# artis-mcrt/artis

Measured on AMD Instinct MI355X. Metric: packet-steps/sec, higher is better.
Workload: dtype f64

## Files before the change

### artis_amd/csrc/artis_engine.hip

```cpp
#include <hip/hip_runtime.h>
#include <rccl/rccl.h>

#include <dlfcn.h>

#include <cstdio>
#include <cstdlib>
#include <algorithm>
#include <chrono>
#include <cstring>
#include <string>
#include <type_traits>
#include <utility>
#include <vector>
#include <cmath>

#include "model_build.h"
#include "engine_config.h"
#include "physics.h"
#include "radfield_fit.h"
#include "ion_balance.h"
#include "spectra.h"

#include <rocprim/device/device_radix_sort.hpp>

// ... 91 lines not shown
  int base = 0;
  for (int w0 = 0; w0 < nw; w0 += 64) {
    const int j = w0 + lane;
    unsigned long long word = (j < nw) ? keep[j] : 0ull;
    const int pc = __popcll(word);
    int incl = pc;
#pragma unroll
    for (int o = 1; o < 64; o <<= 1) {
      const int v = __shfl_up(incl, o);
      if (lane >= o) incl += v;
    }
    int at = base + incl - pc;
    if (j < nw) prefix[j] = at;
    while (word != 0ull) {
      const int i = (j * 64) + __builtin_ctzll(word);
      list[at] = i;
      keptpair[at] = pair[i];
      at++;
      word &= word - 1ull;
    }
    base += __shfl(incl, 63);
  }
}
__global__ void __launch_bounds__(BLOCK) k_corrphotoion(Env env, const int32_t *target_level) {
  const int64_t i = (int64_t)blockIdx.x * BLOCK + threadIdx.x;
  const int64_t total = fill_count(env) * env.M.nphixstargets_total;
  if (i >= total) return;
  const int c = fill_cell(env, i / env.M.nphixstargets_total);
  const int k = (int)(i % env.M.nphixstargets_total);
  const int ul = target_level[k];
  populate_corrphotoion(env, c, ul, k - env.M.level_phixstargetstart[ul]);
}
__device__ inline double wave_shr1(double x) {
  int lo = __double2loint(x), hi = __double2hiint(x);
  lo = __builtin_amdgcn_update_dpp(0, lo, 0x138 , 0xF, 0xF, false);
  hi = __builtin_amdgcn_update_dpp(0, hi, 0x138, 0xF, 0xF, false);
  return __hiloint2double(hi, lo);
}
__device__ inline unsigned long long line_lanes(int lane, int ti, int seglen) {
  const int first = lane - (ti % MAREC_PER);
  const int left = seglen - (ti - (ti % MAREC_PER));
  const int cnt = left < MAREC_PER ? left : MAREC_PER;
  return ((1ull << cnt) - 1ull) << first;
}
struct MaEntryPos {
  LevelPack lpk;
  int ti, seglen, e_seg0;
  bool isdown;
};
__device__ inline MaEntryPos ma_entry_pos(const DevModel &M, int a0, int e) {
  MaEntryPos r;
  r.lpk = M.level_pack[M.alltrans_owner[a0 + e]];
  const int i = (a0 + e) - r.lpk.alltrans_startdown;
  r.isdown = i < r.lpk.ndown;
  r.ti = r.isdown ? i : i - r.lpk.ndown;
  r.seglen = r.isdown ? r.lpk.ndown : r.lpk.nup;
  r.e_seg0 = e - r.ti;
  return r;
}
__global__ void __launch_bounds__(BLOCK, 4) k_matrans(Env env) {
  __shared__ double lds_v[BLOCK / 64][3][MATRANS_BLOCK];
  __shared__ uint16_t lds_q[BLOCK / 64][2][MATRANS_BLOCK];
  __shared__ uint8_t lds_qf[BLOCK / 64][MATRANS_BLOCK];
  __shared__ uint8_t lds_ok[BLOCK / 64][2][MATRANS_BLOCK];
  const int64_t wave = ((int64_t)blockIdx.x * BLOCK + threadIdx.x) >> 6;
  const int lane = threadIdx.x & 63, w = threadIdx.x >> 6;
  const DevModel &M = env.M;
  const int nblk = M.nscanblk;
  if (wave >= fill_count(env) * nblk) return;
  const int64_t kf = wave / nblk;
  const int c = fill_cell(env, kf);
  const int blk = (int)(wave % nblk);
  const int seg0 = M.scanblk_seg0[blk], seg1 = M.scanblk_seg0[blk + 1];
  const MaLongSeg sfirst = M.scansegs[seg0], slast = M.scansegs[seg1 - 1];
  const int a0 = sfirst.ats0, nent = (slast.ats0 + slast.n) - a0;
  U4 *row = env.K.macache + (krow(env, c) * M.nmacache);
  double *upterms = env.collexc_terms + (kf * M.nupcum);
  double(*v)[MATRANS_BLOCK] = lds_v[w];
  if (nent > MATRANS_BLOCK) {
    const LevelPack lpk = M.level_pack[sfirst.ul];
    double c0 = 0., c1 = 0., c2 = 0.;
    for (int base = 0; base < nent; base += 64) {
      const bool valid = base + lane < nent;
      MaTransTerms t;
      t.v0 = t.v1 = t.v2 = t.kterm = 0.;
      if (valid) {
        t = matrans_terms<ARTIS_COLD_COOLING_ONLY != 0>(env, c, a0 + base + lane);
        if (!t.isdown) upterms[M.level_upcum_start[t.ul] + t.i] = t.kterm;
      }
      double s0 = (lane == 0 ? c0 : 0.) + t.v0, s1 = (lane == 0 ? c1 : 0.) + t.v1, s2 = (lane == 0 ? c2 : 0.) + t.v2;
      for (int k = 1; k < 64; k++) {
        const double p0 = wave_shr1(s0), p1 = wave_shr1(s1), p2 = wave_shr1(s2);
        if (lane == k) {
          s0 = p0 + t.v0;
          s1 = p1 + t.v1;
          s2 = p2 + t.v2;
        }
      }
      const int last = (nent - base < 64 ? nent - base : 64) - 1;
      c0 = __shfl(s0, last);
      c1 = __shfl(s1, last);
      c2 = __shfl(s2, last);
    }
    if (lane == 0 && lpk.rec_off >= 0) {
      double *rates = ma_rates_of(row + lpk.rec_off, lpk.ndown, lpk.nup);
      if (sfirst.dir == 0) {
        rates[ARTIS_MA_ACTION_RADDEEXC] = c0;
        rates[ARTIS_MA_ACTION_COLDEEXC] = c1;
        rates[ARTIS_MA_ACTION_INTERNALDOWNSAME] = c2;
      } else {
        rates[ARTIS_MA_ACTION_INTERNALUPSAME] = c0;
      }
    }
    return;
  }
  for (int k = lane; k < nent; k += 64) {
    const int e = M.scanperm[a0 + k];
    const MaTransTerms t = matrans_terms<ARTIS_COLD_COOLING_ONLY != 0>(env, c, a0 + e);
    v[0][e] = t.v0;
    v[1][e] = t.v1;
    v[2][e] = t.v2;
    lds_ok[w][0][e] = 1;
    lds_ok[w][1][e] = 1;
    if (!t.isdown) upterms[M.level_upcum_start[t.ul] + t.i] = t.kterm;
  }
  __threadfence_block();
  for (int si = seg0 + lane; si < seg1; si += 64) {
    const MaLongSeg sg = M.scansegs[si];
    const int o = sg.ats0 - a0;
    double s0 = 0., s1 = 0., s2 = 0.;
    for (int i = 0; i < sg.n; i++) {
      s0 += v[0][o + i];
      s1 += v[1][o + i];
      s2 += v[2][o + i];
      v[0][o + i] = s0;
      v[2][o + i] = s2;
    }
    const LevelPack lpk = M.level_pack[sg.ul];
    if (lpk.rec_off < 0) continue;
    double *rates = ma_rates_of(row + lpk.rec_off, lpk.ndown, lpk.nup);
    if (sg.dir == 0) {
      rates[ARTIS_MA_ACTION_RADDEEXC] = s0;
      rates[ARTIS_MA_ACTION_COLDEEXC] = s1;
      rates[ARTIS_MA_ACTION_INTERNALDOWNSAME] = s2;
    } else {
      rates[ARTIS_MA_ACTION_INTERNALUPSAME] = s0;
    }
  }
  __threadfence_block();
  for (int e = lane; e < nent; e += 64) {
    const MaEntryPos ps = ma_entry_pos(M, a0, e);
    const int e_last = ps.e_seg0 + ps.seglen - 1;
    const double whole_int = v[ps.isdown ? 2 : 0][e_last], whole_rad = v[0][e_last];
    bool ok_int = (whole_int > 0.) && (whole_int <= DBLMAX), ok_rad = (whole_rad > 0.) && (whole_rad <= DBLMAX);
    uint32_t q_int = MAFILT_NONE23, q_rad = MAFILT_NONE;
    if (ps.ti < ps.seglen - 1) {
      if (ok_int) q_int = mafilt_quant23(v[ps.isdown ? 2 : 0][e], whole_int, &ok_int);
      if (ok_rad && ps.isdown) q_rad = mafilt_quant(v[0][e], whole_rad, &ok_rad);
    }
    lds_q[w][0][e] = (uint16_t)(q_int >> 8);
    lds_qf[w][e] = (uint8_t)(q_int & 0xFFu);
    lds_q[w][1][e] = (uint16_t)q_rad;
    const int e_line = e - (ps.ti % MAREC_PER);
    if (!ok_int) lds_ok[w][0][e_line] = 0;
    if (ps.isdown && !ok_rad) lds_ok[w][1][e_line] = 0;
  }
  __threadfence_block();
  for (int e = lane; e < nent; e += 64) {
    const MaEntryPos ps = ma_entry_pos(M, a0, e);
    if (ps.lpk.rec_off < 0) continue;
    const int e_line = e - (ps.ti % MAREC_PER);
    U4 *rec = row + ps.lpk.rec_off;
    const bool lok_int = lds_ok[w][0][e_line] != 0;
    U4 *line = rec + marec_slot(ps.isdown ? MADIR_DOWN : MADIR_UP, ps.ti / MAREC_PER, ps.lpk.ndown, ps.lpk.nup);
    mafilt_put(line, ps.ti % MAREC_PER, lok_int ? lds_q[w][0][e] : 0u);
    ((uint8_t *)rec)[marec_fine_byte0(ps.isdown ? MADIR_DOWN : MADIR_UP, ps.ti / MAREC_PER, ps.lpk.ndown, ps.lpk.nup) + (ps.ti % MAREC_PER)] =
        lok_int ? lds_qf[w][e] : (uint8_t)0u;
    if (ps.ti % MAREC_PER == 0) mafilt_put(line, 7, lok_int ? MAFILT_NONE : 0u);
    if (ps.isdown) {
      const bool lok_rad = lds_ok[w][1][e_line] != 0;
      U4 *rline = rec + marec_slot(MADIR_RAD, ps.ti / MAREC_PER, ps.lpk.ndown, ps.lpk.nup);
      mafilt_put(rline, ps.ti % MAREC_PER, lok_rad ? lds_q[w][1][e] : 0u);
      if (ps.ti % MAREC_PER == 0) mafilt_put(rline, 7, lok_rad ? MAFILT_NONE : 0u);
    }
  }
}
__device__ inline double row_shr1(double x);
__global__ void __launch_bounds__(BLOCK) k_macroatom_recomb(Env env) {
  const int64_t row_id = ((int64_t)blockIdx.x * BLOCK + threadIdx.x) >> 4;
  const int r = threadIdx.x & 15;
  const DevModel &M = env.M;
  const int64_t nrows = fill_count(env) * M.nrecomblevels;
  const bool valid = row_id < nrows;
  const int c = fill_cell(env, (valid ? row_id : 0) / M.nrecomblevels);
  const int ul = M.recomb_levels[(valid ? row_id : 0) % M.nrecomblevels];
  const int ui = M.level_ion[ul];
  const int ls = M.ion_uniquelevelindexstart[ui > 0 ? ui - 1 : 0];
  const int64_t cb = krow(env, c) * M.nphixstargets_total;
  const double e_cur = eps(M, ul);
  const int j0 = valid ? M.level_recomb_start[ul] : 0, j1 = valid ? M.level_recomb_start[ul + 1] : 0;
  double carry0 = 0., carry1 = 0., carry2 = 0.;
  for (int j = j0; __any(j < j1); j += 16) {
    const bool in = (j + r) < j1;
    double x0 = 0., x1 = 0., x2 = 0.;
    if (in) {
      const int lower = M.recomb_lower[j + r];
      const int t = M.recomb_target[j + r];
      const double e_target = eps(M, ls + lower);
// ... 10 lines not shown
    for (int s = 1; s < 16; s++) {
      const double p0 = row_shr1(a0), p1 = row_shr1(a1), p2 = row_shr1(a2);
      if (r == s) {
        a0 = p0 + x0;
        a1 = p1 + x1;
        a2 = p2 + x2;
      }
    }
    const int src = ((threadIdx.x & 63) | 15) << 2;
    carry0 = __hiloint2double(__builtin_amdgcn_ds_bpermute(src, __double2hiint(a0)), __builtin_amdgcn_ds_bpermute(src, __double2loint(a0)));
    carry1 = __hiloint2double(__builtin_amdgcn_ds_bpermute(src, __double2hiint(a1)), __builtin_amdgcn_ds_bpermute(src, __double2loint(a1)));
    carry2 = __hiloint2double(__builtin_amdgcn_ds_bpermute(src, __double2hiint(a2)), __builtin_amdgcn_ds_bpermute(src, __double2loint(a2)));
  }
  if (valid && r == 0) {
    const LevelPack lpk = M.level_pack[ul];
    double *rates = ma_rates_of(ma_rec_of(env, c, lpk), lpk.ndown, lpk.nup);
    rates[ARTIS_MA_ACTION_INTERNALDOWNLOWER] = carry0;
    rates[ARTIS_MA_ACTION_RADRECOMB] = carry1;
    rates[ARTIS_MA_ACTION_COLRECOMB] = carry2;
  }
}
__global__ void __launch_bounds__(BLOCK) k_macroatom(Env env) {
  const int64_t i = (int64_t)blockIdx.x * BLOCK + threadIdx.x;
  const int64_t total = fill_count(env) * env.M.nlevels;
  if (i >= total) return;
  if (env.M.level_pack[i % env.M.nlevels].rec_off < 0) return;
  populate_macroatom<true>(env, fill_cell(env, i / env.M.nlevels), (int)(i % env.M.nlevels));
}
__global__ void __launch_bounds__(BLOCK) k_mafilter_long(Env env) {
  const int64_t wave = ((int64_t)blockIdx.x * BLOCK + threadIdx.x) >> 6;
  const int lane = threadIdx.x & 63;
  const int nseg = env.M.nmalongsegs;
  if (wave >= fill_count(env) * nseg) return;
  const int c = fill_cell(env, wave / nseg);
  const MaLongSeg seg = env.M.malongsegs[wave % nseg];
  const LevelPack lpk = env.M.level_pack[seg.ul];
  U4 *rec = env.K.macache + (krow(env, c) * env.M.nmacache) + lpk.rec_off;
  const double *rates = ma_rates_of(rec, lpk.ndown, lpk.nup);
  const bool down = seg.dir == 0;
  const double whole_int = rates[down ? ARTIS_MA_ACTION_INTERNALDOWNSAME : ARTIS_MA_ACTION_INTERNALUPSAME];
  const double whole_rad = rates[ARTIS_MA_ACTION_RADDEEXC];
  double ca = 0., cb = 0.;
  for (int base = 0; base < seg.n; base += 63) {
    const int ti = base + lane;
    const bool valid = lane < 63 && ti < seg.n;
    double a = 0., b = 0.;
    if (valid) {
      const MaTransTerms t = matrans_terms(env, c, seg.ats0 + ti);
      a = down ? t.v2 : t.v0;
      b = down ? t.v0 : 0.;
// ... 2145 lines not shown
    L->drop_dpop = drop && h.ndpop > 0;
    if (L->drop_dpop) per_cell = per_without;
  }
  L->budget = budget;
  L->per_cell = per_cell;
  const int64_t fit = (int64_t)(budget / (double)(per_cell > 0 ? per_cell : 1));
  if (fit < 1 && cfg.budget_given && cfg.src_budget == CONFIG_STRUCT) {
    g_last_error = "artis_amd_config.cache_budget_bytes (" + std::to_string((long long)budget) + ") cannot hold one row of the cell cache (" + std::to_string(per_cell) + " B)";
    return ARTIS_ERR_ARG;
  }
  L->tile_cells = std::max<int64_t>(1, std::min<int64_t>(ncell_all > 0 ? ncell_all : 1, fit));
  L->ntiles = (int)((ncell_all + L->tile_cells - 1) / L->tile_cells);
  if (L->ntiles < 1) L->ntiles = 1;
  if (ARTIS_OPT_VPKT_ON && L->ntiles > 1) {
    g_last_error = "this build has VPKT_ON and the cell cache does not fit one tile (" + std::to_string(per_cell) + " B per cell x " +
                   std::to_string((long long)ncell_all) + " cells): virtual packets need every cell's row resident";
    return ARTIS_ERR_UNSUPPORTED;
  }
  return ARTIS_OK;
}

int64_t pop_batch_cells(const DevModel &h, int64_t tile_cells, const EngineConfig &cfg) {
  const int64_t per = std::max<int64_t>(1, (int64_t)h.nupcum) * (int64_t)sizeof(double);
  return std::max<int64_t>(1, std::min<int64_t>(tile_cells, (int64_t)cfg.pop_scratch / per));
}
size_t pop_scratch_alloc_bytes(const DevModel &h, int64_t batch) {
  return (size_t)(batch * std::max<int64_t>(1, (int64_t)h.nupcum) * (int64_t)sizeof(double)) + 64;
}

int64_t model_table_bytes(const DevModel &h) {
  int64_t bytes = 0;
#define SZ(f, T, count) bytes += (int64_t)sizeof(T) * std::max<int64_t>(1, (int64_t)(count));
  ARTIS_MODEL_ARRAYS(SZ, h)
#undef SZ
#define SZO(f, T, count) \
  if (h.f) bytes += (int64_t)sizeof(T) * std::max<int64_t>(1, (int64_t)(count));
  ARTIS_MODEL_OPTIONAL_ARRAYS(SZO, h)
#undef SZO
  const int ndim = (h.gridtype == ARTIS_GRID_SPHERICAL1D) ? 1 : ((h.gridtype == ARTIS_GRID_CYLINDRICAL2D) ? 2 : 3);
  for (int a = 0; a < 3; a++) bytes += (int64_t)sizeof(double) * std::max<int64_t>(1, (a >= ndim) ? 1 : h.ncoordgrid[a]);
  bytes += (int64_t)sizeof(int32_t) * std::max<int64_t>(1, h.nphixstargets_total);
  return bytes;
}

struct RcclApi {
  ncclResult_t (*GetUniqueId)(ncclUniqueId *) = nullptr;
  ncclResult_t (*CommInitRank)(ncclComm_t *, int, ncclUniqueId, int) = nullptr;
// ... 551 lines not shown
  if (h.ncold > 0 && (nfill < 0 || !e->pool_keep)) {
    HIP_TRY(hipMemsetAsync(e->K.ma_pool_used, 0, sizeof(uint32_t), s));
    if (nfill >= 0) HIP_TRY(hipMemsetAsync(e->K.ma_rowtab, 0xFF, sizeof(int32_t) * (size_t)(e->tile_cells * (int64_t)h.ncold), s));
  }
  const Env env_tile = env;
  for (int64_t b0 = 0; b0 < ncell_fill; b0 += e->pop_batch) {
  const int64_t ncell = std::min<int64_t>(e->pop_batch, ncell_fill - b0);
  env = env_tile;
  if (nfill >= 0) {
    env.fill_cells = e->d_fill_cells + b0;
    env.nfill = (int32_t)ncell;
  } else {
    env.tile_lo = lo + (int)b0;
    env.tile_hi = lo + (int)(b0 + ncell);
  }
  if (h.ncold > 0) hipLaunchKernelGGL(k_ma_reset, dim3(nblocks(ncell * h.ncold)), dim3(BLOCK), 0, s, env);
  hipLaunchKernelGGL(k_levelpops, dim3(nblocks(ncell * h.nlevels)), dim3(BLOCK), 0, s, env);
  if (h.ndpop > 0) hipLaunchKernelGGL(k_line_dpop, dim3(nblocks(ncell * h.nlines)), dim3(BLOCK), 0, s, env);
  hipLaunchKernelGGL(k_cell_scalars, dim3(nblocks(ncell)), dim3(BLOCK), 0, s, env);
  if (h.nbfcontinua > 0) hipLaunchKernelGGL(k_allcont, dim3(nblocks(ncell * h.nkeepwords * 64)), dim3(BLOCK), 0, s, env);
  if (h.nbfcontinua > 0) hipLaunchKernelGGL(k_keptlist, dim3(nblocks(ncell * 64)), dim3(BLOCK), 0, s, env);
  if (h.nphixstargets_total > 0)
    hipLaunchKernelGGL(k_corrphotoion, dim3(nblocks(ncell * h.nphixstargets_total)), dim3(BLOCK), 0, s, env, e->d_target_level);
  if (h.nalltrans > 0) hipLaunchKernelGGL(k_matrans, dim3(nblocks(ncell * h.nscanblk * 64)), dim3(BLOCK), 0, s, env);
  if (h.nrecomblevels > 0) hipLaunchKernelGGL(k_macroatom_recomb, dim3(nblocks(ncell * (int64_t)h.nrecomblevels * 16)), dim3(BLOCK), 0, s, env);
  hipLaunchKernelGGL(k_macroatom, dim3(nblocks(ncell * h.nlevels)), dim3(BLOCK), 0, s, env);
  if (h.nmalongsegs > 0) hipLaunchKernelGGL(k_mafilter_long, dim3(nblocks(ncell * (int64_t)h.nmalongsegs * 64)), dim3(BLOCK), 0, s, env);
#if ARTIS_EXPOPAC_TABLES
  if (e->expopac_own) {
    hipLaunchKernelGGL(k_expopac, dim3(nblocks((int64_t)ncell * ARTIS_EXPOPAC_NBINS)), dim3(BLOCK), 0, s, env);
    if (ARTIS_OPT_RPKT_BB_THERMALISATION) hipLaunchKernelGGL(k_expopac_planck, dim3(nblocks(ncell)), dim3(BLOCK), 0, s, env);
  }
#endif
  hipLaunchKernelGGL(k_cooling_head, dim3(nblocks((int64_t)ncell * h.nions)), dim3(BLOCK), 0, s, env);
  hipLaunchKernelGGL(k_cooling_chain, dim3(nblocks((int64_t)ncell * h.nions * 16)), dim3(BLOCK), 0, s, env);
  if (h.ncoollines > 0) hipLaunchKernelGGL(k_collexc_filter, dim3(nblocks(ncell * (int64_t)h.ncoollines)), dim3(BLOCK), 0, s, env);
  hipLaunchKernelGGL(k_cooling_tail, dim3(nblocks((int64_t)ncell * h.nions * 16)), dim3(BLOCK), 0, s, env);
  hipLaunchKernelGGL(k_cooling_prefix, dim3(nblocks(ncell)), dim3(BLOCK), 0, s, env);
  if (h.nguide > 0) hipLaunchKernelGGL(k_cool_guide, dim3(nblocks(ncell * h.nguide)), dim3(BLOCK), 0, s, env);
  }
  const int64_t ncell = ncell_fill;
  HIP_TRY(hipGetLastError());
  HIP_TRY(hipStreamSynchronize(s));
  unsigned long long add = (unsigned long long)ncell, cur = 0;
  HIP_TRY(hipMemcpy(&cur, e->d_stats + ARTIS_STAT_UPDATECELL, sizeof(cur), hipMemcpyDeviceToHost));
  cur += add;
  HIP_TRY(hipMemcpy(e->d_stats + ARTIS_STAT_UPDATECELL, &cur, sizeof(cur), hipMemcpyHostToDevice));
  int32_t err = 0;
  HIP_TRY(hipMemcpy(&err, e->d_err, sizeof(err), hipMemcpyDeviceToHost));
  if (err != 0) {
    (void)hipMemset(e->d_err, 0, sizeof(int32_t));
    g_last_error = "cell cache population raised error flag " + std::to_string(err);
    return ARTIS_ERR_NOTCONVERGED;
  }
  e->tile_valid_lo = nfill >= 0 ? -1 : 0;
  return ARTIS_OK;
}

int forget_rows(artis_amd_engine *e, hipStream_t s) {
  if (e->ntiles <= 1) return ARTIS_OK;
  std::fill(e->h_krow.begin(), e->h_krow.end(), -1);
  std::fill(e->h_rowcell.begin(), e->h_rowcell.end(), -1);
  HIP_TRY(hipMemsetAsync(e->d_krow, 0xFF, sizeof(int32_t) * e->h_krow.size(), s));
  if (e->Mh.ncold > 0) {
    HIP_TRY(hipMemsetAsync(e->K.ma_pool_used, 0, sizeof(uint32_t), s));
    HIP_TRY(hipMemsetAsync(e->K.ma_rowtab, 0xFF, sizeof(int32_t) * (size_t)(e->tile_cells * (int64_t)e->Mh.ncold), s));
  }
  return ARTIS_OK;
}

int make_resident(artis_amd_engine *e, const std::vector<int32_t> &want, hipStream_t s, int64_t *nfilled) {
  *nfilled = 0;
// ... 565 lines not shown
  const DevModel &h = e->Mh;
  const int cell = c;
  if (e->ntiles == 1) {
    if (e->tile_valid_lo != 0) {
      int rc = populate_tile(e, nullptr);
      if (rc != ARTIS_OK) return rc;
    }
  } else {
    int64_t nfilled = 0;
    int rc = make_resident(e, std::vector<int32_t>{(int32_t)c}, nullptr, &nfilled);
    if (rc != ARTIS_OK) return rc;
    c = e->h_krow[(size_t)c];
  }
#define DL(dst, f, T, per)                                                                                            \
  if (dst && (per) > 0) HIP_TRY(hipMemcpy(dst, e->K.f + (int64_t)c * (per), sizeof(T) * (size_t)(per), hipMemcpyDeviceToHost));
  DL(levelpops, levelpops, double, h.nlevels)
  if (maprocessrates || matrans) {
    double *d_rates = nullptr, *d_trans = nullptr;
    int32_t *d_bad = nullptr;
    HIP_TRY(hipMalloc((void **)&d_rates, sizeof(double) * (size_t)(h.nlevels * 9 + 1)));
    HIP_TRY(hipMalloc((void **)&d_trans, sizeof(double) * (size_t)(h.nmatransblock + 1)));
    HIP_TRY(hipMalloc((void **)&d_bad, sizeof(int32_t)));
    HIP_TRY(hipMemset(d_bad, 0, sizeof(int32_t)));
    const Env env = make_env(e);
    hipLaunchKernelGGL(k_debug_macache, dim3(nblocks(h.nlevels)), dim3(BLOCK), 0, nullptr, env, cell, d_rates, d_trans, d_bad);
    HIP_TRY(hipGetLastError());
    HIP_TRY(hipDeviceSynchronize());
    int32_t bad = 0;
    HIP_TRY(hipMemcpy(&bad, d_bad, sizeof(bad), hipMemcpyDeviceToHost));
    if (maprocessrates) HIP_TRY(hipMemcpy(maprocessrates, d_rates, sizeof(double) * (size_t)h.nlevels * 9, hipMemcpyDeviceToHost));
    if (matrans) HIP_TRY(hipMemcpy(matrans, d_trans, sizeof(double) * (size_t)h.nmatransblock, hipMemcpyDeviceToHost));
    (void)hipFree(d_rates);
    (void)hipFree(d_trans);
    (void)hipFree(d_bad);
    if (bad != 0) {
      g_last_error = std::to_string(bad) + " filter entries of the cell's macro-atom records differ from the sequential form";
      return ARTIS_ERR_NOTCONVERGED;
    }
  }
  DL(allcont_nnlevel, allcont_nnlevel, double, h.nbfcontinua)
  DL(allcont_departure, allcont_departure, double, h.nbfcontinua)
  DL(allcont_edgepart, allcont_edgepart, double, h.nbfcontinua)
  if (allcont_keepbits && h.nbfcontinua > 0)
    HIP_TRY(hipMemcpy(allcont_keepbits, e->K.allcont_keepbits + (int64_t)c * h.nkeepwords, sizeof(uint64_t) * (size_t)((h.nbfcontinua + 63) / 64),
                      hipMemcpyDeviceToHost));
  DL(corrphotoioncoeff, corrphotoioncoeff, double, h.nphixstargets_total)
// ... 15 lines not shown
```

### artis_amd/csrc/model_build.h

```cpp
#pragma once
#include <algorithm>
#include <cmath>
#include <cstdlib>
#include <cstring>
#include <vector>

#include "tables.h"

namespace artis {

struct ModelOwned {
  std::vector<double> temperature_grid;
  std::vector<int32_t> level_ion;
  std::vector<LinePack> line_pack;
  std::vector<LevelPack> level_pack;
  std::vector<int32_t> level_upcum_start;
  std::vector<int32_t> alltrans_owner;
  std::vector<int32_t> scanblk_seg0;
  std::vector<uint8_t> scanperm;
  std::vector<MaLongSeg> scansegs, malongsegs;
  std::vector<MaTarget> alltrans_target;
  std::vector<uint16_t> alltrans_tlevel16;
  std::vector<CoolLineRef> coollines;
  std::vector<ContPack> cont_pack;
  std::vector<int32_t> expopac_linestart;
  std::vector<int32_t> upcum_coolslot;
  std::vector<int32_t> level_recomb_start, recomb_lower, recomb_target, recomb_levels, ion_cooltail_start, level_coolhi, ion_guideoff, ion_guideshift;
};

#define ARTIS_MODEL_ARRAYS(X, m)                                                   \
  X(temperature_grid, double, (ARTIS_OPT_TABLESIZE + 1))                           \
  X(elem_nions, int32_t, (m).nelements)                                            \
  X(elem_uniqueionindexstart, int32_t, (m).nelements)                              \
  X(elem_lowest_ionstage, int32_t, (m).nelements)                                  \
  X(elem_anumber, int32_t, (m).nelements)                                          \
  X(ion_element, int32_t, (m).nions)                                               \
  X(ion_nlevels, int32_t, (m).nions)                                               \
  X(ion_nlevels_ionising, int32_t, (m).nions)                                      \
  X(ion_maxrecombininglevel, int32_t, (m).nions)                                   \
  X(ion_uniquelevelindexstart, int32_t, (m).nions)                                 \
  X(ion_coolingoffset, int32_t, (m).nions)                                         \
  X(ion_ncoolingterms, int32_t, (m).nions)                                         \
  X(level_epsilon, double, (m).nlevels)                                            \
  X(level_statweight, float, (m).nlevels)                                          \
  X(level_alltrans_startdown, int32_t, (m).nlevels)                                \
  X(level_ndowntrans, int32_t, (m).nlevels)                                        \
  X(level_nuptrans, int32_t, (m).nlevels)                                          \
  X(level_closestgroundlevelcont, int32_t, (m).nlevels)                            \
  X(level_phixsstart, int32_t, (m).nlevels)                                        \
  X(level_nphixstargets, int32_t, (m).nlevels)                                     \
  X(level_phixstargetstart, int32_t, (m).nlevels)                                  \
  X(level_bflist_start, int32_t, (m).nlevels)                                      \
  X(level_matransblock_start, int32_t, (m).nlevels)                                \
  X(level_ion, int32_t, (m).nlevels)                                               \
  X(level_pack, LevelPack, (m).nlevels)                                            \
  X(level_coolhi, int32_t, (m).nlevels)                                            \
  X(ion_guideoff, int32_t, (m).nions)                                              \
  X(ion_guideshift, int32_t, (m).nions)                                            \
  X(level_upcum_start, int32_t, (m).nlevels)                                       \
  X(alltrans_lineindex, int32_t, (m).nalltrans)                                    \
  X(alltrans_targetlevelindex, int32_t, (m).nalltrans)                             \
  X(alltrans_owner, int32_t, (m).nalltrans)                                        \
  X(scansegs, MaLongSeg, ((m).nscansegs > 0 ? (m).nscansegs : 1))                  \
  X(scanblk_seg0, int32_t, ((m).nscanblk + 1))                                     \
  X(scanperm, uint8_t, ((m).nalltrans > 0 ? (m).nalltrans : 1))                    \
  X(malongsegs, MaLongSeg, ((m).nmalongsegs > 0 ? (m).nmalongsegs : 1))            \
  X(alltrans_target, MaTarget, (m).nalltrans)                                      \
  X(alltrans_tlevel16, uint16_t, (((m).nalltrans + 1) & ~1))  \
  X(coollines, CoolLineRef, ((m).ncoollines > 0 ? (m).ncoollines : 1))             \
  X(alltrans_einstein_A, float, (m).nalltrans)                                     \
  X(alltrans_coll_str, float, (m).nalltrans)                                       \
  X(alltrans_osc_strength, float, (m).nalltrans)                                   \
  X(alltrans_forbidden, uint8_t, (m).nalltrans)                                    \
  X(line_nu, double, (m).nlines)                                                   \
  X(line_pack, LinePack, (m).nlines)                                               \
  X(cont_pack, ContPack, (m).nbfcontinua)                                          \
  X(line_elementindex, int32_t, (m).nlines)                                        \
  X(line_ionindex, int32_t, (m).nlines)                                            \
  X(allphixs, float, ((int64_t)(m).nphixslevels * (m).NPHIXSPOINTS))               \
  X(allphixstargets_levelindex, int32_t, (m).nphixstargets_total)                  \
  X(allphixstargets_probability, double, (m).nphixstargets_total)                  \
  X(allcont_nu_edge, double, (m).nbfcontinua)                                      \
  X(allcont_element, int32_t, (m).nbfcontinua)                                     \
  X(allcont_ion, int32_t, (m).nbfcontinua)                                         \
  X(allcont_level, int32_t, (m).nbfcontinua)                                       \
  X(allcont_phixstargetindex, int32_t, (m).nbfcontinua)                            \
  X(allcont_upperlevel, int32_t, (m).nbfcontinua)                                  \
  X(allcont_uniquelevelindex, int32_t, (m).nbfcontinua)                            \
// ... 148 lines not shown
      for (int t = 0; t < lp.ndown + lp.nup; t++) {
        const int tl = m.alltrans_targetlevelindex[lp.alltrans_startdown + t];
        const LevelPack &tp = own.level_pack[start + tl];
        own.alltrans_target[lp.alltrans_startdown + t] = MaTarget{tp.rec_off, tp.alltrans_startdown, tl, (uint32_t)tp.ndown | ((uint32_t)tp.nup << 16)};
      }
    }
  }
  v.alltrans_target = own.alltrans_target.data();
  own.alltrans_tlevel16.assign((size_t)(m.nalltrans > 0 ? ((m.nalltrans + 1) & ~1) : 2), 0);
  for (int i = 0; i < m.nalltrans; i++) own.alltrans_tlevel16[i] = (uint16_t)m.alltrans_targetlevelindex[i];
  v.alltrans_tlevel16 = own.alltrans_tlevel16.data();
  own.level_upcum_start.resize(m.nlevels);
  int32_t nupcum = 0;
  for (int i = 0; i < m.nlevels; i++) {
    own.level_upcum_start[i] = nupcum;
    nupcum += m.level_nuptrans[i];
  }
  v.nupcum = nupcum;
  own.alltrans_owner.assign((size_t)(m.nalltrans > 0 ? m.nalltrans : 1), 0);
  for (int i = 0; i < m.nlevels; i++)
    for (int t = 0; t < m.level_ndowntrans[i] + m.level_nuptrans[i]; t++) own.alltrans_owner[m.level_alltrans_startdown[i] + t] = i;
  v.alltrans_owner = own.alltrans_owner.data();
  {
    own.scansegs.clear();
    own.scanblk_seg0.assign(1, 0);
    own.malongsegs.clear();
    int blk_fill = 0;
    for (int i = 0; i < m.nlevels; i++) {
      const LevelPack &lp = own.level_pack[i];
      for (int dir = 0; dir < 2; dir++) {
        const int n = dir == 0 ? lp.ndown : lp.nup;
        if (n <= 0) continue;
        const int sa = lp.alltrans_startdown + (dir == 0 ? 0 : lp.ndown);
        if (blk_fill > 0 && (blk_fill + n > MATRANS_BLOCK)) {
          own.scanblk_seg0.push_back((int32_t)own.scansegs.size());
          blk_fill = 0;
        }
        own.scansegs.push_back(MaLongSeg{sa, n, i, dir});
        blk_fill += n;
        if (n > MATRANS_BLOCK) {
          if (lp.rec_off >= 0) own.malongsegs.push_back(MaLongSeg{sa, n, i, dir});
          own.scanblk_seg0.push_back((int32_t)own.scansegs.size());
          blk_fill = 0;
        }
      }
    }
    if (blk_fill > 0) own.scanblk_seg0.push_back((int32_t)own.scansegs.size());
    v.nscansegs = (int32_t)own.scansegs.size();
    v.nscanblk = (int32_t)own.scanblk_seg0.size() - 1;
    if (own.scansegs.empty()) own.scansegs.push_back(MaLongSeg{0, 0, 0, 0});
    v.scansegs = own.scansegs.data();
    v.scanblk_seg0 = own.scanblk_seg0.data();
    own.scanperm.assign((size_t)(m.nalltrans > 0 ? m.nalltrans : 1), 0);
    for (int b = 0; b < v.nscanblk; b++) {
      const MaLongSeg &s0 = own.scansegs[own.scanblk_seg0[b]], &s1 = own.scansegs[own.scanblk_seg0[b + 1] - 1];
      const int a0 = s0.ats0, nent = (s1.ats0 + s1.n) - a0;
      if (nent > MATRANS_BLOCK) continue;
      std::vector<int> idx((size_t)nent);
      for (int e = 0; e < nent; e++) idx[e] = e;
      auto kind = [&](int e) {
        const int ati = a0 + e, ul = own.alltrans_owner[ati];
        const bool down = (ati - m.level_alltrans_startdown[ul]) < m.level_ndowntrans[ul];
        const int branch = (m.alltrans_coll_str[ati] < 0) ? (m.alltrans_forbidden[ati] ? 2 : 1) : 0;
        return (down ? 0 : 3) + branch;
      };
      std::stable_sort(idx.begin(), idx.end(), [&](int x, int y) { return kind(x) < kind(y); });
      for (int e = 0; e < nent; e++) own.scanperm[a0 + e] = (uint8_t)idx[e];
    }
    v.scanperm = own.scanperm.data();
    v.nmalongsegs = (int32_t)own.malongsegs.size();
    if (own.malongsegs.empty()) own.malongsegs.push_back(MaLongSeg{0, 0, 0, 0});
    v.malongsegs = own.malongsegs.data();
  }
  v.level_upcum_start = own.level_upcum_start.data();
  own.cont_pack.resize(m.nbfcontinua);
  for (int i = 0; i < m.nbfcontinua; i++)
    own.cont_pack[i] = ContPack{m.allcont_nu_edge[i], m.allcont_probability[i],
                                m.level_phixsstart[m.allcont_uniquelevelindex[i]] * m.NPHIXSPOINTS,
                                m.allcont_groundcontestimindex[i], {0, 0}};
  v.cont_pack = own.cont_pack.data();
  own.expopac_linestart.assign(ARTIS_EXPOPAC_NBINS + 1, m.nlines);
  {
    int li = 0;
    const double nu0 = 1e8 * 2.99792458e+10 / ARTIS_EXPOPAC_LAMBDAMIN;
    while (li < m.nlines && m.line_nu[li] > nu0) li++;
    for (int b = 0; b < ARTIS_EXPOPAC_NBINS; b++) {
      own.expopac_linestart[b] = li;
      const double nu_lower = 1e8 * 2.99792458e+10 / (ARTIS_EXPOPAC_LAMBDAMIN + ((double)(b + 1) * ARTIS_EXPOPAC_DELTALAMBDA));
      while (li < m.nlines && m.line_nu[li] >= nu_lower) li++;
    }
// ... 244 lines not shown
```

### artis_amd/csrc/tables.h

```cpp
#pragma once
#include <stdint.h>

#include "../../include/artis_amd.h"
#include "../../include/artis_options.h"

namespace artis {

struct alignas(16) LinePack {
  int32_t lower;
  int32_t upper;
  float B_ul;
  float B_lu;
};

struct alignas(16) LevelPack {
  int32_t rec_off;
  int32_t alltrans_startdown;
  int32_t ndown;
  int32_t nup;
};
struct alignas(32) ContPack {
  double nu_edge;
  double probability;
  int32_t xs_off;
// ... 14 lines not shown
constexpr int MAREC_PER = 7;
constexpr int MAREC_QUAD = 4;
constexpr int MAREC_RATE_SLOTS = 5;
enum { MADIR_DOWN = 0, MADIR_UP = 1, MADIR_RAD = 2, MADIR_COOL = 3 };
constexpr int marec_lines(int n) { return (n + MAREC_PER - 1) / MAREC_PER; }
constexpr int marec_rest(int n) { return n > MAREC_PER ? marec_lines(n) - 1 : 0; }
constexpr int marec_slot(int d, int l, int nd, int nu) {
  return (d < MADIR_COOL && l == 0)
             ? 1 + d
             : (d == MADIR_DOWN ? MAREC_QUAD + (l - 1)
                                : (d == MADIR_UP ? MAREC_QUAD + marec_rest(nd) + (l - 1)
                                                 : (d == MADIR_RAD ? MAREC_QUAD + marec_rest(nd) + marec_rest(nu) + (l - 1)
                                                                   : MAREC_QUAD + (2 * marec_rest(nd)) + marec_rest(nu) + l)));
}
constexpr int marec_rates_slot(int nd, int nu) { return MAREC_QUAD + (2 * marec_rest(nd)) + marec_rest(nu) + marec_lines(nu); }
constexpr int marec_fine_dirslots(int n) { return (marec_lines(n) + 1) / 2; }
constexpr int marec_fine_slot0(int nd, int nu) { return marec_rates_slot(nd, nu) + MAREC_RATE_SLOTS; }
constexpr int marec_fine_byte0(int d, int l, int nd, int nu) {
  return ((marec_fine_slot0(nd, nu) + (d == MADIR_UP ? marec_fine_dirslots(nd) : 0)) * 16) + (l * 8);
}
constexpr int marec_slots(int nd, int nu) { return marec_fine_slot0(nd, nu) + marec_fine_dirslots(nd) + marec_fine_dirslots(nu); }
constexpr double MAFILT_SCALE = 32768.;
constexpr uint32_t MAFILT_NONE = 0x7FFFu;
constexpr int MATRANS_BLOCK = 256;
constexpr int MAREC_SLACK = 16;

struct alignas(16) D2 {
  double x, y;
};
struct alignas(16) MaLongSeg {
  int32_t ats0, n, ul, dir;
};
struct alignas(8) CoolLineRef {
  int32_t slot, up0, first, n, cool_hi, cool_lo;
};

struct VpktConfig;
struct DevModel {
  int32_t nelements, nions, nlevels, nlines, nalltrans, nphixstargets_total, nphixslevels, nbfcontinua, nbfcontinua_ground,
      ncoolingterms, nmatransblock, NPHIXSPOINTS;
  int32_t nmacache;
  int32_t ncold, ma_pool_slots;
  const int32_t *level_coolhi;
  int32_t nguide, guide_ion_shift;
  const int32_t *ion_guideoff, *ion_guideshift;
  int32_t nupcum;
  int32_t ndpop;
// ... 19 lines not shown
  const int32_t *allcont_bfestimindex;
  int32_t nbfestim;
  const float *rho_tmin;
  const int32_t *xcom_elem_start;
  const double *xcom_energy, *xcom_sigma;
  int32_t nxcom;
  const int32_t *detailed_lineindices;
  int32_t detailed_linecount;
  const VpktConfig *vpkt;
  const int32_t *ion_element, *ion_nlevels, *ion_nlevels_ionising, *ion_maxrecombininglevel, *ion_uniquelevelindexstart,
      *ion_coolingoffset, *ion_ncoolingterms;
  const double *level_epsilon;
  const float *level_statweight;
  const int32_t *level_alltrans_startdown, *level_ndowntrans, *level_nuptrans, *level_closestgroundlevelcont, *level_phixsstart,
      *level_nphixstargets, *level_phixstargetstart, *level_bflist_start, *level_matransblock_start;
  const int32_t *level_ion;
  const LevelPack *level_pack;
  const int32_t *level_upcum_start;
  const int32_t *alltrans_lineindex, *alltrans_targetlevelindex;
  const int32_t *alltrans_owner;
  const MaLongSeg *scansegs;
  const int32_t *scanblk_seg0;
  int32_t nscansegs, nscanblk;
  const uint8_t *scanperm;
  const MaLongSeg *malongsegs;
  int32_t nmalongsegs;
  const MaTarget *alltrans_target;
  const uint16_t *alltrans_tlevel16;
  const CoolLineRef *coollines;
  int32_t ncoollines;
  const float *alltrans_einstein_A, *alltrans_coll_str, *alltrans_osc_strength;
  const uint8_t *alltrans_forbidden;
  const double *line_nu;
  const LinePack *line_pack;
  const ContPack *cont_pack;
  const int32_t *line_elementindex, *line_ionindex;
  const float *allphixs;
  const int32_t *allphixstargets_levelindex;
  const double *allphixstargets_probability;
  const double *allcont_nu_edge;
  const int32_t *allcont_element, *allcont_ion, *allcont_level, *allcont_phixstargetindex, *allcont_upperlevel,
      *allcont_uniquelevelindex, *allcont_groundcontestimindex;
  const double *allcont_probability;
  const double *groundcont_nu_edge;
  const double *spontrecombcoeffs, *corrphotoioncoeffs, *bfcooling_coeffs;
  const uint8_t *coolinglist_type;
  const int32_t *coolinglist_level, *coolinglist_phixstargetindex;
// ... 135 lines not shown
```

### artis_amd/synth.py

```python
from __future__ import annotations

import numpy as np

from . import abi

CLIGHT = 2.99792458e10
H = 6.6260755e-27
KB = 1.38064852e-16
EV = 1.6021772e-12
ME = 9.1093897e-28
QE = 4.80325e-10
MH = 1.67352e-24
MSUN = 1.98855e33
DAY = 86400.0
SAHACONST = 2.0706659e-16
CLIGHTSQUAREDOVERTWOH = CLIGHT**2 / (2 * H)
TABLESIZE = 100
MINTEMP = 3500.0
MAXTEMP = 140000.0
MINPOP = 1e-30

_IONPOT = {
    8: [13.62, 35.12, 54.94, 77.41, 113.9],
    14: [8.15, 16.35, 33.49, 45.14, 166.8],
# ... 55 lines not shown
            ion_element.append(e)
            ion_nlevels.append(nl)
            ion_uls.append(len(level_eps))
            ion_ionpot.append(ionpot)
            for k in range(nl):
                level_eps.append(eps_ground + E[k])
                level_g.append(float(rng.integers(1, 11)))
                level_ion.append(nions_total)
            eps_ground += ionpot
            nions_total += 1
    nlevels = len(level_eps)
    level_eps = np.array(level_eps)
    level_g = np.array(level_g, dtype=np.float32)
    ion_uls = np.array(ion_uls, dtype=np.int32)
    ion_nlevels = np.array(ion_nlevels, dtype=np.int32)
    ion_element = np.array(ion_element, dtype=np.int32)

    lines = []
    for ui in range(nions_total):
        nl = ion_nlevels[ui]
        s = ion_uls[ui]
        for lo in range(nl):
            for up in range(lo + 1, nl):
                if rng.random() >= line_fraction:
                    continue
                dE = level_eps[s + up] - level_eps[s + lo]
                nu = dE / H
                if nu < 2e13:
                    continue
                forb = rng.random() < forbidden_fraction
                A = 10 ** rng.uniform(-2, 2) if forb else 10 ** rng.uniform(5.0, 8.5) * min(1.0, (dE / (5 * EV)) ** 2)
                cs = rng.uniform(0.1, 5.0) if rng.random() < collstr_fraction else -1.0
                lines.append((nu, ui, lo, up, A, cs, forb))
    lines.sort(key=lambda t: -t[0])
    nlines = len(lines)
    line_nu = np.array([t[0] for t in lines])
    line_ui = np.array([t[1] for t in lines], dtype=np.int32)
    line_lo = np.array([t[2] for t in lines], dtype=np.int32)
    line_up = np.array([t[3] for t in lines], dtype=np.int32)
    line_A = np.array([t[4] for t in lines], dtype=np.float32)
    line_cs = np.array([t[5] for t in lines], dtype=np.float32)
    line_forb = np.array([t[6] for t in lines], dtype=np.uint8)
    line_ul_lower = ion_uls[line_ui] + line_lo
    line_ul_upper = ion_uls[line_ui] + line_up
    line_nu = (level_eps[line_ul_upper] - level_eps[line_ul_lower]) / H
    order = np.argsort(-line_nu, kind="stable")
    (line_nu, line_ui, line_lo, line_up, line_A, line_cs, line_forb, line_ul_lower, line_ul_upper) = (
# ... 723 lines not shown
```

Before: 1.367 billion.

## Restructure matrans to one block per scan block and fuse macroatom finish

k_matrans now runs one workgroup of MATRANS_THREADS per scan block instead of one wave, with a larger MATRANS_BLOCK (1024) and __syncthreads between phases. Levels that fit wholly in a scan block have populate_macroatom run inside k_matrans, so k_macroatom only handles the leftover levels. The host-side stat update and error readback become a tiny device kernel plus one async copy, replacing several synchronous memcpys. The risks are lower occupancy from the bigger LDS footprint per block, idle threads in the long-segment path, and extra model-build complexity.

```diff
diff --git a/artis_amd/csrc/artis_engine.hip b/artis_amd/csrc/artis_engine.hip
--- a/artis_amd/csrc/artis_engine.hip
+++ b/artis_amd/csrc/artis_engine.hip
@@ -137,6 +137,7 @@
     base += __shfl(incl, 63);
   }
 }
+__global__ void k_stat_add(unsigned long long *stat, unsigned long long add) { *stat += add; }
 __global__ void __launch_bounds__(BLOCK) k_corrphotoion(Env env, const int32_t *target_level) {
   const int64_t i = (int64_t)blockIdx.x * BLOCK + threadIdx.x;
   const int64_t total = fill_count(env) * env.M.nphixstargets_total;
@@ -173,26 +174,24 @@
   r.e_seg0 = e - r.ti;
   return r;
 }
-__global__ void __launch_bounds__(BLOCK, 4) k_matrans(Env env) {
-  __shared__ double lds_v[BLOCK / 64][3][MATRANS_BLOCK];
-  __shared__ uint16_t lds_q[BLOCK / 64][2][MATRANS_BLOCK];
-  __shared__ uint8_t lds_qf[BLOCK / 64][MATRANS_BLOCK];
-  __shared__ uint8_t lds_ok[BLOCK / 64][2][MATRANS_BLOCK];
-  const int64_t wave = ((int64_t)blockIdx.x * BLOCK + threadIdx.x) >> 6;
-  const int lane = threadIdx.x & 63, w = threadIdx.x >> 6;
+__global__ void __launch_bounds__(MATRANS_THREADS) k_matrans(Env env) {
+  __shared__ double v[3][MATRANS_BLOCK];
+  __shared__ uint16_t lds_q[2][MATRANS_BLOCK];
+  __shared__ uint8_t lds_qf[MATRANS_BLOCK];
+  __shared__ uint8_t lds_ok[2][MATRANS_BLOCK];
+  const int tid = threadIdx.x, lane = threadIdx.x & 63;
   const DevModel &M = env.M;
   const int nblk = M.nscanblk;
-  if (wave >= fill_count(env) * nblk) return;
-  const int64_t kf = wave / nblk;
+  const int64_t kf = (int64_t)blockIdx.x / nblk;
   const int c = fill_cell(env, kf);
-  const int blk = (int)(wave % nblk);
+  const int blk = (int)((int64_t)blockIdx.x % nblk);
   const int seg0 = M.scanblk_seg0[blk], seg1 = M.scanblk_seg0[blk + 1];
   const MaLongSeg sfirst = M.scansegs[seg0], slast = M.scansegs[seg1 - 1];
   const int a0 = sfirst.ats0, nent = (slast.ats0 + slast.n) - a0;
   U4 *row = env.K.macache + (krow(env, c) * M.nmacache);
   double *upterms = env.collexc_terms + (kf * M.nupcum);
-  double(*v)[MATRANS_BLOCK] = lds_v[w];
   if (nent > MATRANS_BLOCK) {
+    if (tid >= 64) return;
     const LevelPack lpk = M.level_pack[sfirst.ul];
     double c0 = 0., c1 = 0., c2 = 0.;
     for (int base = 0; base < nent; base += 64) {
@@ -229,18 +228,18 @@
     }
     return;
   }
-  for (int k = lane; k < nent; k += 64) {
+  for (int k = tid; k < nent; k += MATRANS_THREADS) {
     const int e = M.scanperm[a0 + k];
     const MaTransTerms t = matrans_terms<ARTIS_COLD_COOLING_ONLY != 0>(env, c, a0 + e);
     v[0][e] = t.v0;
     v[1][e] = t.v1;
     v[2][e] = t.v2;
-    lds_ok[w][0][e] = 1;
-    lds_ok[w][1][e] = 1;
+    lds_ok[0][e] = 1;
+    lds_ok[1][e] = 1;
     if (!t.isdown) upterms[M.level_upcum_start[t.ul] + t.i] = t.kterm;
   }
-  __threadfence_block();
-  for (int si = seg0 + lane; si < seg1; si += 64) {
+  __syncthreads();
+  for (int si = seg0 + tid; si < seg1; si += MATRANS_THREADS) {
     const MaLongSeg sg = M.scansegs[si];
     const int o = sg.ats0 - a0;
     double s0 = 0., s1 = 0., s2 = 0.;
@@ -262,8 +261,8 @@
       rates[ARTIS_MA_ACTION_INTERNALUPSAME] = s0;
     }
   }
-  __threadfence_block();
-  for (int e = lane; e < nent; e += 64) {
+  __syncthreads();
+  for (int e = tid; e < nent; e += MATRANS_THREADS) {
     const MaEntryPos ps = ma_entry_pos(M, a0, e);
     const int e_last = ps.e_seg0 + ps.seglen - 1;
     const double whole_int = v[ps.isdown ? 2 : 0][e_last], whole_rad = v[0][e_last];
@@ -273,32 +272,39 @@
       if (ok_int) q_int = mafilt_quant23(v[ps.isdown ? 2 : 0][e], whole_int, &ok_int);
       if (ok_rad && ps.isdown) q_rad = mafilt_quant(v[0][e], whole_rad, &ok_rad);
     }
-    lds_q[w][0][e] = (uint16_t)(q_int >> 8);
-    lds_qf[w][e] = (uint8_t)(q_int & 0xFFu);
-    lds_q[w][1][e] = (uint16_t)q_rad;
+    lds_q[0][e] = (uint16_t)(q_int >> 8);
+    lds_qf[e] = (uint8_t)(q_int & 0xFFu);
+    lds_q[1][e] = (uint16_t)q_rad;
     const int e_line = e - (ps.ti % MAREC_PER);
-    if (!ok_int) lds_ok[w][0][e_line] = 0;
-    if (ps.isdown && !ok_rad) lds_ok[w][1][e_line] = 0;
-  }
-  __threadfence_block();
-  for (int e = lane; e < nent; e += 64) {
+    if (!ok_int) lds_ok[0][e_line] = 0;
+    if (ps.isdown && !ok_rad) lds_ok[1][e_line] = 0;
+  }
+  __syncthreads();
+  for (int e = tid; e < nent; e += MATRANS_THREADS) {
     const MaEntryPos ps = ma_entry_pos(M, a0, e);
     if (ps.lpk.rec_off < 0) continue;
     const int e_line = e - (ps.ti % MAREC_PER);
     U4 *rec = row + ps.lpk.rec_off;
-    const bool lok_int = lds_ok[w][0][e_line] != 0;
+    const bool lok_int = lds_ok[0][e_line] != 0;
     U4 *line = rec + marec_slot(ps.isdown ? MADIR_DOWN : MADIR_UP, ps.ti / MAREC_PER, ps.lpk.ndown, ps.lpk.nup);
-    mafilt_put(line, ps.ti % MAREC_PER, lok_int ? lds_q[w][0][e] : 0u);
+    mafilt_put(line, ps.ti % MAREC_PER, lok_int ? lds_q[0][e] : 0u);
     ((uint8_t *)rec)[marec_fine_byte0(ps.isdown ? MADIR_DOWN : MADIR_UP, ps.ti / MAREC_PER, ps.lpk.ndown, ps.lpk.nup) + (ps.ti % MAREC_PER)] =
-        lok_int ? lds_qf[w][e] : (uint8_t)0u;
+        lok_int ? lds_qf[e] : (uint8_t)0u;
     if (ps.ti % MAREC_PER == 0) mafilt_put(line, 7, lok_int ? MAFILT_NONE : 0u);
     if (ps.isdown) {
-      const bool lok_rad = lds_ok[w][1][e_line] != 0;
+      const bool lok_rad = lds_ok[1][e_line] != 0;
       U4 *rline = rec + marec_slot(MADIR_RAD, ps.ti / MAREC_PER, ps.lpk.ndown, ps.lpk.nup);
-      mafilt_put(rline, ps.ti % MAREC_PER, lok_rad ? lds_q[w][1][e] : 0u);
+      mafilt_put(rline, ps.ti % MAREC_PER, lok_rad ? lds_q[1][e] : 0u);
       if (ps.ti % MAREC_PER == 0) mafilt_put(rline, 7, lok_rad ? MAFILT_NONE : 0u);
     }
   }
+#if ARTIS_MATRANS_FINISH
+  for (int ul = M.scanblk_lev0[blk] + tid; ul < M.scanblk_lev0[blk + 1]; ul += MATRANS_THREADS) {
+    const LevelPack lpk = M.level_pack[ul];
+    if (lpk.rec_off < 0 || lpk.ndown + lpk.nup > MATRANS_BLOCK) continue;
+    populate_macroatom<true>(env, c, ul);
+  }
+#endif
 }
 __device__ inline double row_shr1(double x);
 __global__ void __launch_bounds__(BLOCK) k_macroatom_recomb(Env env) {
@@ -355,10 +361,11 @@
 }
 __global__ void __launch_bounds__(BLOCK) k_macroatom(Env env) {
   const int64_t i = (int64_t)blockIdx.x * BLOCK + threadIdx.x;
-  const int64_t total = fill_count(env) * env.M.nlevels;
+  const int64_t total = fill_count(env) * env.M.nmaleft;
   if (i >= total) return;
-  if (env.M.level_pack[i % env.M.nlevels].rec_off < 0) return;
-  populate_macroatom<true>(env, fill_cell(env, i / env.M.nlevels), (int)(i % env.M.nlevels));
+  const int ul = env.M.maleft_levels[i % env.M.nmaleft];
+  if (env.M.level_pack[ul].rec_off < 0) return;
+  populate_macroatom<true>(env, fill_cell(env, i / env.M.nmaleft), ul);
 }
 __global__ void __launch_bounds__(BLOCK) k_mafilter_long(Env env) {
   const int64_t wave = ((int64_t)blockIdx.x * BLOCK + threadIdx.x) >> 6;
@@ -2550,7 +2557,8 @@
 
 int64_t pop_batch_cells(const DevModel &h, int64_t tile_cells, const EngineConfig &cfg) {
   const int64_t per = std::max<int64_t>(1, (int64_t)h.nupcum) * (int64_t)sizeof(double);
-  return std::max<int64_t>(1, std::min<int64_t>(tile_cells, (int64_t)cfg.pop_scratch / per));
+  const int64_t grid_cells = (int64_t)INT32_MAX / std::max<int64_t>(1, (int64_t)h.nscanblk);
+  return std::max<int64_t>(1, std::min<int64_t>(std::min<int64_t>(tile_cells, grid_cells), (int64_t)cfg.pop_scratch / per));
 }
 size_t pop_scratch_alloc_bytes(const DevModel &h, int64_t batch) {
   return (size_t)(batch * std::max<int64_t>(1, (int64_t)h.nupcum) * (int64_t)sizeof(double)) + 64;
@@ -3148,9 +3156,9 @@
   if (h.nbfcontinua > 0) hipLaunchKernelGGL(k_keptlist, dim3(nblocks(ncell * 64)), dim3(BLOCK), 0, s, env);
   if (h.nphixstargets_total > 0)
     hipLaunchKernelGGL(k_corrphotoion, dim3(nblocks(ncell * h.nphixstargets_total)), dim3(BLOCK), 0, s, env, e->d_target_level);
-  if (h.nalltrans > 0) hipLaunchKernelGGL(k_matrans, dim3(nblocks(ncell * h.nscanblk * 64)), dim3(BLOCK), 0, s, env);
   if (h.nrecomblevels > 0) hipLaunchKernelGGL(k_macroatom_recomb, dim3(nblocks(ncell * (int64_t)h.nrecomblevels * 16)), dim3(BLOCK), 0, s, env);
-  hipLaunchKernelGGL(k_macroatom, dim3(nblocks(ncell * h.nlevels)), dim3(BLOCK), 0, s, env);
+  if (h.nalltrans > 0) hipLaunchKernelGGL(k_matrans, dim3((unsigned)(ncell * h.nscanblk)), dim3(MATRANS_THREADS), 0, s, env);
+  if (h.nmaleft > 0) hipLaunchKernelGGL(k_macroatom, dim3(nblocks(ncell * (int64_t)h.nmaleft)), dim3(BLOCK), 0, s, env);
   if (h.nmalongsegs > 0) hipLaunchKernelGGL(k_mafilter_long, dim3(nblocks(ncell * (int64_t)h.nmalongsegs * 64)), dim3(BLOCK), 0, s, env);
 #if ARTIS_EXPOPAC_TABLES
   if (e->expopac_own) {
@@ -3165,15 +3173,11 @@
   hipLaunchKernelGGL(k_cooling_prefix, dim3(nblocks(ncell)), dim3(BLOCK), 0, s, env);
   if (h.nguide > 0) hipLaunchKernelGGL(k_cool_guide, dim3(nblocks(ncell * h.nguide)), dim3(BLOCK), 0, s, env);
   }
-  const int64_t ncell = ncell_fill;
+  hipLaunchKernelGGL(k_stat_add, dim3(1), dim3(1), 0, s, e->d_stats + ARTIS_STAT_UPDATECELL, (unsigned long long)ncell_fill);
   HIP_TRY(hipGetLastError());
+  HIP_TRY(hipMemcpyAsync(e->h_counts, e->d_count, sizeof(int32_t) * (2 * NEXT_NKINDS + 1), hipMemcpyDeviceToHost, s));
   HIP_TRY(hipStreamSynchronize(s));
-  unsigned long long add = (unsigned long long)ncell, cur = 0;
-  HIP_TRY(hipMemcpy(&cur, e->d_stats + ARTIS_STAT_UPDATECELL, sizeof(cur), hipMemcpyDeviceToHost));
-  cur += add;
-  HIP_TRY(hipMemcpy(e->d_stats + ARTIS_STAT_UPDATECELL, &cur, sizeof(cur), hipMemcpyHostToDevice));
-  int32_t err = 0;
-  HIP_TRY(hipMemcpy(&err, e->d_err, sizeof(err), hipMemcpyDeviceToHost));
+  const int32_t err = e->h_counts[2 * NEXT_NKINDS];
   if (err != 0) {
     (void)hipMemset(e->d_err, 0, sizeof(int32_t));
     g_last_error = "cell cache population raised error flag " + std::to_string(err);
@@ -3785,6 +3789,8 @@
     HIP_TRY(hipMalloc((void **)&d_trans, sizeof(double) * (size_t)(h.nmatransblock + 1)));
     HIP_TRY(hipMalloc((void **)&d_bad, sizeof(int32_t)));
     HIP_TRY(hipMemset(d_bad, 0, sizeof(int32_t)));
+    HIP_TRY(hipMemset(d_rates, 0, sizeof(double) * (size_t)(h.nlevels * 9 + 1)));
+    HIP_TRY(hipMemset(d_trans, 0, sizeof(double) * (size_t)(h.nmatransblock + 1)));
     const Env env = make_env(e);
     hipLaunchKernelGGL(k_debug_macache, dim3(nblocks(h.nlevels)), dim3(BLOCK), 0, nullptr, env, cell, d_rates, d_trans, d_bad);
     HIP_TRY(hipGetLastError());
diff --git a/artis_amd/csrc/model_build.h b/artis_amd/csrc/model_build.h
--- a/artis_amd/csrc/model_build.h
+++ b/artis_amd/csrc/model_build.h
@@ -16,8 +16,8 @@
   std::vector<LevelPack> level_pack;
   std::vector<int32_t> level_upcum_start;
   std::vector<int32_t> alltrans_owner;
-  std::vector<int32_t> scanblk_seg0;
-  std::vector<uint8_t> scanperm;
+  std::vector<int32_t> scanblk_seg0, scanblk_lev0, maleft_levels;
+  std::vector<uint16_t> scanperm;
   std::vector<MaLongSeg> scansegs, malongsegs;
   std::vector<MaTarget> alltrans_target;
   std::vector<uint16_t> alltrans_tlevel16;
@@ -63,7 +63,9 @@
   X(alltrans_owner, int32_t, (m).nalltrans)                                        \
   X(scansegs, MaLongSeg, ((m).nscansegs > 0 ? (m).nscansegs : 1))                  \
   X(scanblk_seg0, int32_t, ((m).nscanblk + 1))                                     \
-  X(scanperm, uint8_t, ((m).nalltrans > 0 ? (m).nalltrans : 1))                    \
+  X(scanblk_lev0, int32_t, ((m).nscanblk + 1))                                     \
+  X(maleft_levels, int32_t, ((m).nmaleft > 0 ? (m).nmaleft : 1))                   \
+  X(scanperm, uint16_t, ((m).nalltrans > 0 ? (m).nalltrans : 1))                   \
   X(malongsegs, MaLongSeg, ((m).nmalongsegs > 0 ? (m).nmalongsegs : 1))            \
   X(alltrans_target, MaTarget, (m).nalltrans)                                      \
   X(alltrans_tlevel16, uint16_t, (((m).nalltrans + 1) & ~1))  \
@@ -258,12 +260,20 @@
     for (int t = 0; t < m.level_ndowntrans[i] + m.level_nuptrans[i]; t++) own.alltrans_owner[m.level_alltrans_startdown[i] + t] = i;
   v.alltrans_owner = own.alltrans_owner.data();
   {
+    const bool finish = ARTIS_MATRANS_FINISH != 0 && v.ncold == 0;
     own.scansegs.clear();
     own.scanblk_seg0.assign(1, 0);
     own.malongsegs.clear();
+    std::vector<int32_t> home((size_t)m.nlevels, 0);
     int blk_fill = 0;
     for (int i = 0; i < m.nlevels; i++) {
       const LevelPack &lp = own.level_pack[i];
+      const bool whole = finish && lp.ndown + lp.nup <= MATRANS_BLOCK;
+      if (whole && blk_fill > 0 && blk_fill + lp.ndown + lp.nup > MATRANS_BLOCK) {
+        own.scanblk_seg0.push_back((int32_t)own.scansegs.size());
+        blk_fill = 0;
+      }
+      home[(size_t)i] = (int32_t)own.scanblk_seg0.size() - 1;
       for (int dir = 0; dir < 2; dir++) {
         const int n = dir == 0 ? lp.ndown : lp.nup;
         if (n <= 0) continue;
@@ -271,6 +281,7 @@
         if (blk_fill > 0 && (blk_fill + n > MATRANS_BLOCK)) {
           own.scanblk_seg0.push_back((int32_t)own.scansegs.size());
           blk_fill = 0;
+          if (dir == 0) home[(size_t)i] = (int32_t)own.scanblk_seg0.size() - 1;
         }
         own.scansegs.push_back(MaLongSeg{sa, n, i, dir});
         blk_fill += n;
@@ -287,6 +298,25 @@
     if (own.scansegs.empty()) own.scansegs.push_back(MaLongSeg{0, 0, 0, 0});
     v.scansegs = own.scansegs.data();
     v.scanblk_seg0 = own.scanblk_seg0.data();
+    own.scanblk_lev0.assign((size_t)v.nscanblk + 1, m.nlevels);
+    own.maleft_levels.clear();
+    for (int i = 0, b = 0; i < m.nlevels && v.nscanblk > 0 && finish; i++)
+      for (const int h = std::min<int>(home[(size_t)i], v.nscanblk - 1); b <= h; b++) own.scanblk_lev0[(size_t)b] = i;
+    for (int i = 0; i < m.nlevels; i++) {
+      const LevelPack &lp = own.level_pack[i];
+      if (lp.rec_off < 0) continue;
+      bool left = !finish || v.nscanblk == 0 || lp.ndown + lp.nup > MATRANS_BLOCK;
+      if (!left) {
+        const int b = std::min<int>(home[(size_t)i], v.nscanblk - 1);
+        const MaLongSeg &s0 = own.scansegs[own.scanblk_seg0[b]], &s1 = own.scansegs[own.scanblk_seg0[b + 1] - 1];
+        left = (s1.ats0 + s1.n) - s0.ats0 > MATRANS_BLOCK;
+      }
+      if (left) own.maleft_levels.push_back(i);
+    }
+    v.nmaleft = (int32_t)own.maleft_levels.size();
+    if (own.maleft_levels.empty()) own.maleft_levels.push_back(0);
+    v.scanblk_lev0 = own.scanblk_lev0.data();
+    v.maleft_levels = own.maleft_levels.data();
     own.scanperm.assign((size_t)(m.nalltrans > 0 ? m.nalltrans : 1), 0);
     for (int b = 0; b < v.nscanblk; b++) {
       const MaLongSeg &s0 = own.scansegs[own.scanblk_seg0[b]], &s1 = own.scansegs[own.scanblk_seg0[b + 1] - 1];
@@ -301,7 +331,7 @@
         return (down ? 0 : 3) + branch;
       };
       std::stable_sort(idx.begin(), idx.end(), [&](int x, int y) { return kind(x) < kind(y); });
-      for (int e = 0; e < nent; e++) own.scanperm[a0 + e] = (uint8_t)idx[e];
+      for (int e = 0; e < nent; e++) own.scanperm[a0 + e] = (uint16_t)idx[e];
     }
     v.scanperm = own.scanperm.data();
     v.nmalongsegs = (int32_t)own.malongsegs.size();
diff --git a/artis_amd/csrc/tables.h b/artis_amd/csrc/tables.h
--- a/artis_amd/csrc/tables.h
+++ b/artis_amd/csrc/tables.h
@@ -60,7 +60,15 @@
 constexpr int marec_slots(int nd, int nu) { return marec_fine_slot0(nd, nu) + marec_fine_dirslots(nd) + marec_fine_dirslots(nu); }
 constexpr double MAFILT_SCALE = 32768.;
 constexpr uint32_t MAFILT_NONE = 0x7FFFu;
-constexpr int MATRANS_BLOCK = 256;
+#ifndef ARTIS_MATRANS_BLOCK
+#define ARTIS_MATRANS_BLOCK 1024
+#endif
+#ifndef ARTIS_MATRANS_FINISH
+#define ARTIS_MATRANS_FINISH 1
+#endif
+constexpr int MATRANS_BLOCK = ARTIS_MATRANS_BLOCK;
+constexpr int MATRANS_THREADS = MATRANS_BLOCK / 4;
+static_assert(MATRANS_BLOCK <= 65536 && MATRANS_THREADS >= 64 && MATRANS_THREADS <= 1024 && MATRANS_THREADS % 64 == 0, "k_matrans block");
 constexpr int MAREC_SLACK = 16;
 
 struct alignas(16) D2 {
@@ -126,7 +134,10 @@
   const MaLongSeg *scansegs;
   const int32_t *scanblk_seg0;
   int32_t nscansegs, nscanblk;
-  const uint8_t *scanperm;
+  const int32_t *scanblk_lev0;
+  const int32_t *maleft_levels;
+  int32_t nmaleft;
+  const uint16_t *scanperm;
   const MaLongSeg *malongsegs;
   int32_t nmalongsegs;
   const MaTarget *alltrans_target;
diff --git a/artis_amd/synth.py b/artis_amd/synth.py
--- a/artis_amd/synth.py
+++ b/artis_amd/synth.py
@@ -101,7 +101,7 @@
         s = ion_uls[ui]
         for lo in range(nl):
             for up in range(lo + 1, nl):
-                if rng.random() >= line_fraction:
+                if rng.random() >= (line_fraction(lo, up) if callable(line_fraction) else line_fraction):
                     continue
                 dE = level_eps[s + up] - level_eps[s + lo]
                 nu = dE / H
```

Result: faster. 1.383 billion (median of 6 runs) (+1.2%).
